# travisturner/pilosa

Hardware: AMD Instinct MI355X
Metric: PQL queries/sec (Count(Intersect(Row,Row))) on 1M-row x 1B-col set field (higher is better)
Workload: dtype bitmap(u64 words); 1 GPU; model=set field f, 1M-row x 1B-col (954 shards), global_batch=4096, seq_len=1000000000, parallelism=shard-range x1

## Files before the change

### pilosa_amd/kernels/binding.cpp

```cpp
#include <ATen/hip/HIPContext.h>
#include <torch/extension.h>

#include <pybind11/numpy.h>
#include <pybind11/stl.h>

#include <algorithm>
#include <cstring>
#include <mutex>
#include <vector>

#include "kernels.h"

namespace {

void check_dev(const torch::Tensor& t, const char* name) {
  TORCH_CHECK(t.is_cuda(), name, " must be a device tensor");
  TORCH_CHECK(t.is_contiguous(), name, " must be contiguous");
}

hipStream_t cur_stream(const torch::Tensor& t) {
  return at::hip::getCurrentHIPStream(t.device().index()).stream();
}

void check_launch(const char* what) {
// ... 340 lines not shown
  b.view = int32_t(a[0]);
  b.depth = int32_t(a[1]);
  TORCH_CHECK(b.depth >= 0 && b.depth <= 63, "bsi depth");
  TORCH_CHECK(a[0] >= 0 && a[0] < views.numel() / int64_t(sizeof(pk::ViewDev)), "bsi view slot");
  TORCH_CHECK(planes >= 1 && planes <= 64 && gchunk >= 1 && gchunk < (int64_t(1) << 31), "bsi_group_sum: slab / chunk");
  b.row_exists = a[2];
  b.row_sign = a[3];
  for (int i = 0; i < 64; i++) b.bit_row[i] = i < 63 ? a[4 + i] : -1;
  const int nslab = pk::launch_bsi_group_sum(
      reinterpret_cast<const pk::QueryProg*>(progs.data_ptr<uint8_t>()), int(G),
      reinterpret_cast<const pk::ViewDev*>(views.data_ptr<uint8_t>()), int(S), b, int(planes), int(gchunk),
      int(fmode), reinterpret_cast<unsigned long long*>(out_sum.data_ptr<int64_t>()),
      reinterpret_cast<unsigned long long*>(out_cnt.data_ptr<int64_t>()), cur_stream(progs));
  TORCH_CHECK(nslab >= 0, "bsi_group_sum: grid too large");
  check_launch("bsi_group_sum");
  return nslab;
}

void and2_count(torch::Tensor progs, torch::Tensor views, int64_t S, torch::Tensor pairs, torch::Tensor partial,
                int64_t cq, int64_t variant) {
  check_dev(progs, "progs");
  check_dev(views, "views");
  check_dev(pairs, "pairs");
  check_dev(partial, "partial");
  const int Q = int(progs.numel() / sizeof(pk::QueryProg));
  const int64_t n = int64_t(Q) * S * 16;
  TORCH_CHECK(pairs.numel() * pairs.element_size() >= n * 8, "pairs scratch must hold S*16*Q uint2");
  TORCH_CHECK(partial.scalar_type() == torch::kInt32 && partial.numel() >= n, "partial must be int32[S*16*Q]");
  pk::launch_and2_pairs(reinterpret_cast<const pk::QueryProg*>(progs.data_ptr<uint8_t>()), Q,
                        reinterpret_cast<const pk::ViewDev*>(views.data_ptr<uint8_t>()), int(S),
                        reinterpret_cast<uint2*>(pairs.data_ptr()), partial.data_ptr<int32_t>(), int(cq),
                        int(variant), cur_stream(progs));
  check_launch("and2_pairs");
}

pk::ViewDev viewdev_from(const torch::Tensor& vd);

void twin_build(torch::Tensor view, int64_t S, torch::Tensor rows, torch::Tensor twin) {
  check_dev(rows, "rows");
  check_dev(twin, "twin");
  TORCH_CHECK(rows.scalar_type() == torch::kInt32, "rows must be int32[R]");
  const int64_t R = rows.numel();
  TORCH_CHECK(R >= 0 && R < (int64_t(1) << 20) && S > 0, "twin_build sizes");
  TORCH_CHECK(twin.scalar_type() == torch::kInt64 && twin.numel() == R * S * 16 * 1024,
              "twin must be int64[R*S*16*1024]");
  pk::ViewDev v = viewdev_from(view);
  pk::launch_twin_build(v, int(S), rows.data_ptr<int32_t>(), int(R), reinterpret_cast<uint64_t*>(twin.data_ptr<int64_t>()),
                          cur_stream(twin));
  check_launch("twin_build");
}

void partial_sum_scatter(torch::Tensor partial, int64_t U, int64_t n, torch::Tensor ti, torch::Tensor out) {
  check_dev(partial, "partial");
  check_dev(ti, "ti");
  check_dev(out, "out");
  TORCH_CHECK(partial.scalar_type() == torch::kInt32 && partial.is_contiguous() && partial.numel() >= U * n,
              "partial must be int32[U*n]");
  TORCH_CHECK(ti.scalar_type() == torch::kInt64 && ti.numel() == n, "ti must be int64[n]");
  TORCH_CHECK(out.scalar_type() == torch::kInt64, "out must be int64");
  TORCH_CHECK(n < (int64_t(1) << 31) && U < (int64_t(1) << 40), "partial_sum_scatter sizes");
  pk::launch_partial_sum_scatter(partial.data_ptr<int32_t>(), U, int(n), ti.data_ptr<int64_t>(),
                                 out.data_ptr<int64_t>(), out.numel(), cur_stream(partial));
  check_launch("partial_sum_scatter");
}

pk::ViewDev viewdev_from(const torch::Tensor& vd) {
// ... 653 lines not shown
  const pk::ViewDev v = viewdev_from(view);
  check_dev(out, "out");
  TORCH_CHECK(out.scalar_type() == torch::kInt64, "out int64[n]");
  TORCH_CHECK(unit.dim() == 2 && unit.size(0) == 1, "block_dump takes one unit");
  if (out.numel() == 0) return;
  const torch::Tensor du = checked_units(unit, v, S, M, e, rows);
  pk::launch_block_dump(v, du.data_ptr<int32_t>(), int(M), int(e), rows.data_ptr<int64_t>(),
                        reinterpret_cast<uint64_t*>(out.data_ptr<int64_t>()), out.numel(), cur_stream(rows));
  check_launch("block_dump");
}

}

PYBIND11_MODULE(TORCH_EXTENSION_NAME, m) {
  m.doc() = "gfx950 HIP kernels for the bitmap index";
  m.attr("QUERYPROG_BYTES") = int(sizeof(pk::QueryProg));
  m.attr("VIEWDEV_BYTES") = int(sizeof(pk::ViewDev));
  m.attr("PAIR_VARIANTS") = std::vector<int>{63};
  m.attr("MAXLEAF") = pk::MAXLEAF;
  m.attr("MAXPROG") = pk::MAXPROG;
  m.def("expr_count", &expr_count, "batched boolean-expression count over all local shards",
        py::arg("progs"), py::arg("views"), py::arg("S"), py::arg("out"), py::arg("per_key"), py::arg("mode") = 0,
        py::arg("per_shard") = py::none());
  m.def("expr_materialize", &expr_materialize, "write result containers for a batch of expressions");
#ifdef PK_KBENCH
  m.attr("KBENCH") = true;
#else
  m.attr("KBENCH") = false;
#endif
  m.def("partial_sum_scatter", &partial_sum_scatter, "out[ti[q]] += column sums of int32[U][n] partials");
  m.def("and2_count", &and2_count, "Count(Intersect(a,b)) batch via key-major pair kernels", py::arg("progs"),
        py::arg("views"), py::arg("S"), py::arg("pairs"), py::arg("partial"), py::arg("cq") = 0,
        py::arg("variant") = 1);
  m.def("bsi_range", &bsi_range, "BSI predicate -> bitmap container per (shard, key)");
  m.def("bsi_range_count", &bsi_range_count, "Count(Row(v <op> x)): fused BSI predicate + count");
  m.def("bsi_minmax", &bsi_minmax, "BSI min/max descents per (shard, key); which: 0 both, 1 Min, 2 Max",
        py::arg("progs"), py::arg("views"), py::arg("S"), py::arg("bsi_args"), py::arg("out"), py::arg("which") = 0);
  m.def("bsi_kth_init", &bsi_kth_init, "Percentile: candidate tiles (exists & filter) and N, Nneg");
  m.def("bsi_kth_steps", &bsi_kth_steps, "Percentile: one descent launch per bit, MSB first");
  m.def("bsi_kth_replay", &bsi_kth_replay, "Percentile: host replay of the bit counts -> (magnitude, count)");
  m.def("bsi_distinct", &bsi_distinct, "Distinct: mark the magnitudes of exists & filter in the pos / neg bitmaps");
  m.def("distinct_slots", [](int64_t depth, int64_t want) { return int64_t(pk::distinct_slots(int(depth), int(want))); },
        "Distinct: tile slots per workgroup the launcher uses for this depth and request");
  m.def("leaf_src", &leaf_src, "src containers of plain rows straight from the arena (TopN srcs)");
  m.def("row_counts", &row_counts, "row counts of (shard, dense row) entries (device rank caches)");
  m.def("topn_cache_counts", &topn_cache_counts, "cache-only TopN: [candidate x shard] row counts");
  m.def("topn_cache_batch", &topn_cache_batch, "cache-only TopN batch: membership, totals, per-query top-n");
  m.def("mesh_cache_issue", &mesh_cache_issue, "mesh cache-only TopN share: params, partial buffer (pre all-reduce)");
  m.def("mesh_cache_finish", &mesh_cache_finish, "mesh cache-only TopN: select, D2H, decode (post all-reduce)");
  py::class_<CacheTopN>(m, "CacheTopN")
      .def(py::init<torch::Tensor, torch::Tensor, torch::Tensor, torch::Tensor, int64_t, torch::Tensor>())
      .def("run", &CacheTopN::run, "cache-only TopN batch end to end: (ids, counts, offsets) or None")
      .def_property_readonly("U", &CacheTopN::U)
      .def_property_readonly("stride", &CacheTopN::stride);
  m.def("upload_i32", &upload_i32, "small host int32 array -> device through a pinned ring (current stream)");
  m.def("topn_cache_partial", &topn_cache_partial, "mesh cache-only TopN: one rank's membership + partial totals");
  m.def("topn_cache_select32", &topn_cache_select32, "mesh cache-only TopN: per-query top-n of the reduced buffer");
  m.def("row_counts_sum", &row_counts_sum, "ids= re-count without src: per id the sum of shard row counts >= threshold");
  m.def("twin_build", &twin_build, "bitmap twins of dense array rows for the pair kernels");
  m.def("keymask_build", &keymask_build, "key-presence mask of every (shard, row) of a view");
  m.def("topn_hot_meta", &topn_hot_meta, "key-j container of every hot cache rank of the TopN index");
  m.def("topn_index", &topn_index, "build pass of the device TopN slot index (count or fill)");
  m.def("bsi_minmax_fold", &bsi_minmax_fold, "fold BSI min/max descents into one (value, count, found)");
  m.def("topn_src", &topn_src, "src-filtered TopN over the slot index: mode 1 heap walk, mode 2/3 ids= re-count (rebuilt / kept histograms)");
  m.def("bitgemm", &bitgemm, "row-pair intersection count matrix of dense bit rows (mode 1 MFMA i8, 0 VALU); "
        "c_split_stride > 0: one matrix per K-split; skip_lower: no tiles below the diagonal (A is B)",
        py::arg("A"), py::arg("B"), py::arg("M"), py::arg("N"), py::arg("KW"), py::arg("splits"), py::arg("mode"),
// ... 24 lines not shown
```

### pilosa_amd/kernels/kernels.h

```cpp
#pragma once
#include <hip/hip_runtime.h>
#include <stdint.h>

namespace pk {

constexpr int MAXLEAF = 16;
constexpr int MAXPROG = 32;
constexpr int ARRAY_MAX = 4096;
constexpr int RUN_MAX = 2048;
constexpr int CT_ARRAY = 1, CT_BITMAP = 2, CT_RUN = 3;
constexpr int OP_AND = 32, OP_OR = 33, OP_XOR = 34, OP_ANDNOT = 35;

__host__ __device__ __forceinline__ int meta_j(int64_t m) { return int(m & 15); }
__host__ __device__ __forceinline__ int meta_type(int64_t m) { return int((m >> 4) & 3); }
__host__ __device__ __forceinline__ int meta_n(int64_t m) { return int((m >> 6) & 0x1ffff); }
__host__ __device__ __forceinline__ int64_t meta_off16(int64_t m) { return int64_t(uint64_t(m) >> 23); }

struct QueryProg {
  int32_t nleaf;
  int32_t nprog;
  int32_t leaf_view[MAXLEAF];
  int64_t leaf_row[MAXLEAF];
  uint8_t prog[MAXPROG];
  int64_t pad[3];
// ... 5 lines not shown
  const int64_t* shard_base;
  const int64_t* meta;
  const uint16_t* payload;
  int64_t D;
  const uint16_t* keymask;
  uint64_t reserved0;
  uint64_t reserved1;
  const uint64_t* twin;
  const int32_t* twin_slot;
  int64_t twin_cutoff;
  const int32_t* hot_counts;
  const int32_t* hot_slot;
  const uint8_t* hot_valid;
  int64_t hot_h;
};
static_assert(sizeof(ViewDev) == 120, "ViewDev layout");

struct BsiArgs {
  int32_t view;
  int32_t depth;
  int64_t row_exists;
  int64_t row_sign;
  int64_t bit_row[64];
};

void launch_expr_count(const QueryProg* progs, int Q, const ViewDev* views, int S, unsigned long long* out,
                       int32_t* per_key, int64_t* per_shard, int mode, hipStream_t st);
void launch_expr_materialize(const QueryProg* progs, int Q, const ViewDev* views, int S, const int32_t* counts,
                             const int64_t* offs, uint16_t* outp, hipStream_t st);
void launch_partial_sum_scatter(const int32_t* partial, int64_t U, int n, const int64_t* ti, int64_t* out,
                                int64_t nout, hipStream_t st);
void launch_and2_pairs(const QueryProg* progs, int Q, const ViewDev* views, int S, uint2* pairs, int32_t* partial,
                       int cq, int variant, hipStream_t st);
void launch_bsi_range(const ViewDev* views, int S, BsiArgs bsi, int op, int64_t p1, int64_t p2, uint16_t* out_payload,
                      int64_t* out_meta, unsigned long long* out_count, hipStream_t st);
void launch_bsi_minmax_fold(const int64_t* o, int F, int G, int is_min, int64_t* out, int64_t* part,
                            hipStream_t st);
void launch_bsi_minmax(const QueryProg* progs, const ViewDev* views, int S, BsiArgs bsi, int64_t* out,
                       hipStream_t st, int which = 0);
__host__ __device__ inline int kth_chain(int largest_first, uint64_t c1, uint64_t& r, uint64_t& tot) {
  const uint64_t c0 = tot - c1;
  if (largest_first) {
    if (r < c1) { tot = c1; return 1; }
    r -= c1; tot = c0; return 0;
  }
  if (r < c0) { tot = c0; return 0; }
  r -= c0; tot = c1; return 1;
}
constexpr int KTH_CNT = 2 + 64;
void launch_bsi_kth_init(const QueryProg* progs, const ViewDev* views, int S, BsiArgs bsi, uint64_t* cand,
                         unsigned long long* cnt, hipStream_t st);
void launch_bsi_kth_step(const ViewDev* views, int S, BsiArgs bsi, uint64_t* cand, unsigned long long* cnt, int i,
                         uint64_t r, uint64_t tot, int largest_first, hipStream_t st);
void launch_bsi_sum(const QueryProg* progs, int Q, const ViewDev* views, int S, BsiArgs bsi,
                    unsigned long long* out_sum, unsigned long long* out_cnt, int fmode, hipStream_t st);
constexpr int GS_MAX_PLANES = 13;
int launch_bsi_group_sum(const QueryProg* progs, int G, const ViewDev* views, int S, BsiArgs bsi, int planes,
                         int gchunk, int fmode, unsigned long long* out_sum, unsigned long long* out_cnt,
                         hipStream_t st);

constexpr int DISTINCT_MAX_PLANES = 32;
int distinct_slots(int depth, int want);
int launch_bsi_distinct(const QueryProg* progs, const ViewDev* views, int S, BsiArgs bsi, int slots, int mark,
                        uint32_t* pos, uint32_t* neg, hipStream_t st);

int64_t launch_row_filter_counts(const ViewDev& fv, const ViewDev* xv, int64_t xd, int S, int64_t rows_per_block,
// ... 86 lines not shown
```

### pilosa_amd/kernels/pair_kernels.hip

```cpp
#include <hip/hip_runtime.h>
#include <stdint.h>

#include "kernels.h"
#include "device_util.h"

namespace pk {
namespace {

constexpr uint32_t NONE = 0xffffffffu;
constexpr uint32_t PRECOUNTED = 0xfffffffeu;

__global__ __launch_bounds__(256) void keymask_build_kernel(ViewDev v, int S, uint16_t* __restrict__ out) {
  const int64_t t = int64_t(blockIdx.x) * blockDim.x + threadIdx.x;
  if (t >= int64_t(S) * v.D) return;
  const int s = int(t / v.D);
  const int64_t d = t - int64_t(s) * v.D;
  v.keymask = nullptr;
  int64_t lo;
  out[t] = uint16_t(row_keys(v, s, d, lo));
}

__global__ __launch_bounds__(256) void pair_build_kernel(const QueryProg* __restrict__ progs, int Q,
                                                         const ViewDev* __restrict__ views, int S,
                                                         uint2* __restrict__ pairs, int hot) {
  const int64_t t = int64_t(blockIdx.x) * blockDim.x + threadIdx.x;
  if (t >= int64_t(Q) * S) return;
  const int s = int(t / Q), q = int(t % Q);
  const QueryProg& qp = progs[q];
  uint2* dst = pairs + int64_t(s) * 16 * Q + q;
  if (hot && qp.leaf_view[0] == qp.leaf_view[1] && qp.leaf_row[0] >= 0 && qp.leaf_row[1] >= 0) {
    const ViewDev& hv = views[qp.leaf_view[0]];
    if (hv.hot_counts != nullptr && gp(hv.hot_valid)[s]) {
      const int sa = gp(hv.hot_slot)[qp.leaf_row[0]], sb = gp(hv.hot_slot)[qp.leaf_row[1]];
      if (sa >= 0 && sb >= 0) {
        const int64_t h = hv.hot_h;
        const uint32_t c = uint32_t(gp(hv.hot_counts)[(int64_t(s) * h + min(sa, sb)) * h + max(sa, sb)]);
        dst[0] = make_uint2(PRECOUNTED, c);
#pragma unroll
        for (int j = 1; j < 16; j++) dst[int64_t(j) * Q] = make_uint2(NONE, NONE);
        return;
      }
    }
  }
  int64_t loa, lob;
  const uint32_t pa = row_keys(views[qp.leaf_view[0]], s, qp.leaf_row[0], loa);
  const uint32_t pb = row_keys(views[qp.leaf_view[1]], s, qp.leaf_row[1], lob);
  const uint32_t both = pa & pb;
#pragma unroll
  for (int j = 0; j < 16; j++) {
    uint2 e = make_uint2(NONE, NONE);
    if ((both >> j) & 1) {
      const uint32_t below = (1u << j) - 1;
      e.x = uint32_t(loa + __popc(pa & below));
      e.y = uint32_t(lob + __popc(pb & below));
    }
    dst[int64_t(j) * Q] = e;
  }
}


__device__ __forceinline__ void lds_clear(uint64_t* lb) {
  ulong2* l2 = reinterpret_cast<ulong2*>(lb);
  const int lane = wave_lane();
#pragma unroll
  for (int i = 0; i < 8; i++) l2[i * 64 + lane] = make_ulong2(0, 0);
}

template <bool BST = false>
__device__ __forceinline__ void stage(uint64_t* lb, const uint16_t* p, int64_t m) {
  const int lane = wave_lane();
  const int type = meta_type(m);
  ulong2* l2 = reinterpret_cast<ulong2*>(lb);
  if (type == CT_BITMAP) {
    const auto g = gp(reinterpret_cast<const ulong2*>(p));
    ulong2 t[8];
#pragma unroll
    for (int i = 0; i < 8; i++) t[i] = g[i * 64 + lane];
#pragma unroll
    for (int i = 0; i < 8; i++) l2[i * 64 + lane] = t[i];
    lds_fence();
    return;
  }
  uint32_t* l32 = reinterpret_cast<uint32_t*>(lb);
  if (BST && type == CT_ARRAY) {
    const int n = meta_n(m);
    const auto p4 = gp(reinterpret_cast<const uint4*>(p));
    const int n8 = (n + 7) >> 3;
    bool cleared = false;
    for (int b = 0; b < n8; b += 4 * 64) {
      uint4 v[4];
// ... 287 lines not shown
  const int lane = wave_lane();
  ulong2* dst = reinterpret_cast<ulong2*>(twin + w * 1024);
  const int64_t d = rows[r];
  int64_t c = -1;
  if (d >= 0) {
    int64_t lo;
    const uint32_t pres = row_keys(v, s, d, lo);
    if ((pres >> j) & 1) c = lo + __popc(pres & ((1u << j) - 1));
  }
  if (c < 0) {
#pragma unroll
    for (int i = 0; i < 8; i++) dst[i * 64 + lane] = make_ulong2(0, 0);
    return;
  }
  const int64_t m = gp(v.meta)[c];
  stage<true>(lb, payload_of(v, m), m);
  const ulong2* l2 = reinterpret_cast<const ulong2*>(lb);
#pragma unroll
  for (int i = 0; i < 8; i++) dst[i * 64 + lane] = l2[i * 64 + lane];
}

__device__ __forceinline__ int64_t meta_as_bitmap(int64_t m) {
  return (m & ~(int64_t(3) << 4)) | (int64_t(CT_BITMAP) << 4);
}

__device__ __forceinline__ void twin_swap(const ViewDev& v, int64_t d, int S, int64_t u, int64_t& m, uint64_t& pl) {
  if (v.twin_slot == nullptr || meta_type(m) != CT_ARRAY || meta_n(m) <= v.twin_cutoff) return;
  const int sl = gp(v.twin_slot)[d];
  if (sl < 0) return;
  pl = reinterpret_cast<uint64_t>(v.twin + ((int64_t(sl) * S + (u >> 4)) * 16 + (u & 15)) * 1024);
  m = meta_as_bitmap(m);
}

template <int CQ, bool BST = false, int TWN = 0>
__global__ __launch_bounds__(64, 5) void and2_pairs_v6_kernel(const QueryProg* __restrict__ progs, int Q,
                                                             const ViewDev* __restrict__ views, int S,
                                                             const uint2* __restrict__ pairs,
                                                             int32_t* __restrict__ partial) {
  __shared__ uint64_t lb[1024];
  const int lane = wave_lane();
  const int64_t gw = int64_t(xcd_remap(blockIdx.x, gridDim.x));
  const int nch = (Q + CQ - 1) / CQ;
  const int64_t u = gw / nch;
  if (u >= int64_t(S) * 16) return;
  const int q0 = int(gw % nch) * CQ;
  const int nq = min(CQ, Q - q0);

  uint32_t ea = NONE;
  int vai = -1;
  int64_t ma = 0, mb = 0;
  uint64_t pal = 0, pbl = 0;
  int mine = 0;
  if (lane < nq) {
    const uint2 e = pairs[u * Q + q0 + lane];
    if (e.x == PRECOUNTED) {
      mine = int(e.y);
    } else if (e.x != NONE) {
      ea = e.x;
      vai = progs[q0 + lane].leaf_view[0];
      const int vbi = progs[q0 + lane].leaf_view[1];
      ma = gp(views[vai].meta)[e.x];
      mb = gp(views[vbi].meta)[e.y];
      pal = reinterpret_cast<uint64_t>(payload_of(views[vai], ma));
      pbl = reinterpret_cast<uint64_t>(payload_of(views[vbi], mb));
      if (TWN & 1) twin_swap(views[vai], progs[q0 + lane].leaf_row[0], S, u, ma, pal);
      if (TWN & 2) twin_swap(views[vbi], progs[q0 + lane].leaf_row[1], S, u, mb, pbl);
    }
  }
  uint64_t todo = __ballot(ea != NONE);
  if (todo) {
    uint32_t cached = NONE;
    int cached_v = -1;
    int i = __builtin_ctzll(todo);
    todo &= todo - 1;
// ... 11 lines not shown
      int c = 0;
      if (a == cached && va == cached_v) {
        c = count_vs_head(lb, pB, mB, head);
      } else {
        const bool next_same = j >= 0 && __builtin_amdgcn_readlane(ea, j) == a &&
                               __builtin_amdgcn_readlane(vai, j) == va;
        if (!next_same && tA == CT_BITMAP && tB == CT_BITMAP) {
          c = and_global_bitmaps(reinterpret_cast<const uint64_t*>(pA), reinterpret_cast<const uint64_t*>(pB));
        } else if (!next_same && tA == CT_ARRAY && tB == CT_BITMAP && meta_n(mA) <= SMALL_ARRAY_N) {
          c = probe_small(gp(reinterpret_cast<const uint32_t*>(pB)), pA, meta_n(mA));
        } else if (!next_same && tA == CT_ARRAY && tB == CT_BITMAP) {
          lds_fence();
          stage<BST>(lb, pB, mB);
          cached = NONE;
          cached_v = -1;
          c = count_vs_lds(lb, pA, mA);
        } else {
          lds_fence();
          stage<BST>(lb, pA, mA);
          cached = a;
          cached_v = va;
          c = count_vs_head(lb, pB, mB, head);
        }
      }
      c = wave_sum(c);
      if (lane == i) mine = c;
      if (j < 0) break;
      i = j;
      todo &= todo - 1;
    }
  }
  if (lane < nq) partial[u * Q + q0 + lane] = mine;
}
}

void launch_twin_build(const ViewDev& v, int S, const int32_t* rows, int R, uint64_t* twin, hipStream_t st) {
  const int64_t w = int64_t(R) * S * 16;
  if (w <= 0) return;
  const dim3 grid(unsigned(w < 65535 ? w : 65535), unsigned((w + 65534) / 65535));
  hipLaunchKernelGGL(twin_build_kernel, grid, dim3(64), 0, st, v, S, rows, R, twin);
}

void launch_keymask_build(const ViewDev& v, int S, uint16_t* out, hipStream_t st) {
  const int64_t n = int64_t(S) * v.D;
  if (n == 0) return;
  hipLaunchKernelGGL(keymask_build_kernel, dim3(unsigned((n + 255) / 256)), dim3(256), 0, st, v, S, out);
}

template <int CQ, bool BST, int TWN>
void launch_v6(const QueryProg* progs, int Q, const ViewDev* views, int S, const uint2* pairs, int32_t* partial,
               hipStream_t st) {
  const int64_t wv = int64_t(S) * 16 * ((Q + CQ - 1) / CQ);
  hipLaunchKernelGGL((and2_pairs_v6_kernel<CQ, BST, TWN>), dim3(unsigned(wv)), dim3(64), 0, st, progs, Q, views, S,
                     pairs, partial);
}

void launch_and2_pairs(const QueryProg* progs, int Q, const ViewDev* views, int S, uint2* pairs, int32_t* partial,
                       int cq, int variant, hipStream_t st) {
  const int64_t items = int64_t(Q) * S;
  if (items == 0) return;
  const bool twin = variant == 63 && (cq > 0 ? cq == 64 : Q > 2048);
  if (variant == 63 && !twin) variant = 6;
  if (variant == 6 && cq <= 0 && Q <= 128) {
    variant = 39;
    cq = Q <= 32 ? 4 : (Q <= 64 ? 32 : 16);
  }
  if (cq <= 0) cq = Q <= 128 ? 8 : (Q <= 2048 ? 32 : 64);
  const int hot = variant == 6 || variant == 39 || variant == 63;
  hipLaunchKernelGGL(pair_build_kernel, dim3(unsigned((items + 255) / 256)), dim3(256), 0, st, progs, Q, views, S,
                     pairs, hot);
#define PK_LAUNCH(CQV)                                                         \
  if (variant == 39)                                                           \
    launch_v6<CQV, true, 0>(progs, Q, views, S, pairs, partial, st);           \
  else                                                                         \
    launch_v6<CQV, false, 0>(progs, Q, views, S, pairs, partial, st);          \
  break;
  switch (twin ? 0 : cq) {
    case 0: launch_v6<64, false, 3>(progs, Q, views, S, pairs, partial, st); break;
    case 4: PK_LAUNCH(4)
    case 8: PK_LAUNCH(8)
    case 16: PK_LAUNCH(16)
    case 32: PK_LAUNCH(32)
    default: PK_LAUNCH(64)
  }
#undef PK_LAUNCH
}

__global__ __launch_bounds__(256) void partial_sum_scatter_kernel(const int32_t* __restrict__ partial, int64_t U,
                                                                  int n, const int64_t* __restrict__ ti,
                                                                  unsigned long long* __restrict__ out,
                                                                  int64_t nout) {
  __shared__ long long acc[4][64];
  const int tx = threadIdx.x & 63, ty = threadIdx.x >> 6;
  const int q = int(blockIdx.x) * 64 + tx;
  const int64_t r0 = int64_t(blockIdx.y) * 128;
  const int64_t r1 = r0 + 128 < U ? r0 + 128 : U;
  long long a = 0;
  if (q < n) {
#pragma unroll 8
    for (int64_t r = r0 + ty; r < r1; r += 4) a += partial[r * n + q];
  }
  acc[ty][tx] = a;
  __syncthreads();
  if (ty == 0 && q < n) {
    const long long t = acc[0][tx] + acc[1][tx] + acc[2][tx] + acc[3][tx];
    const int64_t o = ti[q];
    if (t && o >= 0 && o < nout) atomicAdd(out + o, (unsigned long long)t);
  }
}

void launch_partial_sum_scatter(const int32_t* partial, int64_t U, int n, const int64_t* ti, int64_t* out,
                                int64_t nout, hipStream_t st) {
  if (U <= 0 || n <= 0) return;
  const dim3 grid(unsigned((n + 63) / 64), unsigned((U + 127) / 128));
  hipLaunchKernelGGL(partial_sum_scatter_kernel, grid, dim3(256), 0, st, partial, U, n, ti,
                     reinterpret_cast<unsigned long long*>(out), nout);
}

}
```

### pilosa_amd/ops/device.py

```python
from __future__ import annotations

import math
import os
import threading
import time
from dataclasses import dataclass, field
from typing import Dict, List, Optional, Sequence, Tuple

import numpy as np

from pilosa_amd.utils import tracing

MAXLEAF = 16
MAXPROG = 32
OP_AND, OP_OR, OP_XOR, OP_ANDNOT = 32, 33, 34, 35
KIND_AND2, KIND_ROW, KIND_GENERIC, KIND_FLAT, KIND_UNION = 0, 1, 2, 3, 4
KIND_ALIAS = 5
_KERNEL_MODE = {KIND_ROW: 1, KIND_GENERIC: 0, KIND_FLAT: 2, KIND_UNION: 3}


def flat_mask(progs: np.ndarray) -> np.ndarray:
    pg = progs["prog"].astype(np.int32)
    n = progs["nprog"].astype(np.int64)
    pos = np.arange(pg.shape[1])
# ... 1055 lines not shown

def hot_table_passable(table_rows_gen: int, table_gen: int, rows_gen: int, generation: int) -> bool:
    return table_rows_gen == rows_gen and table_gen == generation


def hot_stale_shards(snapshot: np.ndarray, shard_gen: np.ndarray) -> np.ndarray:
    return np.flatnonzero(np.asarray(snapshot) != np.asarray(shard_gen)).astype(np.int64)


def shard_runs(shards, block: int):
    out = []
    for s in np.asarray(shards, np.int64).tolist():
        if out and out[-1][1] == s and s - out[-1][0] < block:
            out[-1][1] = s + 1
        else:
            out.append([s, s + 1])
    return [(a, b) for a, b in out]



class DeviceRowBlock:

    __slots__ = ("shards", "counts", "offs", "payload", "spill")

    def __init__(self, shards, counts, offs, payload, spill=None):
        self.shards, self.counts, self.offs, self.payload, self.spill = list(shards), counts, offs, payload, spill

    def host(self):
        return (self.counts.cpu().numpy(), self.offs.cpu().numpy(), self.payload.cpu().numpy().view(np.uint16))


class GpuEngine:

    def __init__(self, device):
        import torch

        self.torch = torch
        self.device = torch.device(device)
        self.ext = kernels()
        self.copy_stream = torch.cuda.Stream(self.device) if self.device.type == "cuda" else None
        self.use_and2 = os.environ.get("PILOSA_AND2", "1") != "0"
        self.and2_cq = int(os.environ.get("PILOSA_AND2_CQ", "0"))
        self.and2_variant = int(os.environ.get("PILOSA_AND2_VARIANT", "6"))
        built = set(getattr(kernels(), "PAIR_VARIANTS", ()))
        self.use_twin = os.environ.get("PILOSA_TWIN", "1") != "0" and 63 in built
        self.use_hot = os.environ.get("PILOSA_HOTPAIR", "1") != "0"
        self.use_union = os.environ.get("PILOSA_UNION_KERNEL", "1") != "0"
        self.union_variant = int(os.environ.get("PILOSA_UNION_VARIANT", "2"))

    def _and2_aux(self, views: List["DeviceView"], n: int) -> int:
        if self.use_hot and self.and2_variant in (6, 39, 63):
            for v in views:
                v.ensure_hot()
        wave64 = self.and2_cq == 64 or (self.and2_cq <= 0 and n > 2048)
        if self.use_twin and wave64 and self.and2_variant in (6, 63) and \
                any([v.ensure_twin() for v in views]):
            return 2
        return 0

    def _views_tensor(self, views: List["DeviceView"]):
        arr = np.zeros(len(views), dtype=VIEWDEV_DTYPE)
        for i, v in enumerate(views):
            arr[i] = v.viewdev(hot=self.use_hot)
        key = arr.tobytes()
        memo = self.__dict__.setdefault("_vt_memo", {})
        hit = memo.get(key)
        torch = self.torch
        cuda = self.device.type == "cuda"
        if hit is not None:
            t, ev = hit
            if cuda:
                cur = torch.cuda.current_stream(self.device)
                cur.wait_event(ev)
                t.record_stream(cur)
            return t
        t = self._h2d(arr.view(np.uint8))
        ev = None
        if cuda:
            ev = torch.cuda.Event()
# ... 83 lines not shown
            is_row = is_row | is_and2
            is_and2 = np.zeros_like(is_and2)
        flat = flat_mask(progs)
        kind = np.where(is_and2, KIND_AND2, np.where(is_row, KIND_ROW,
                                                      np.where(flat, KIND_FLAT, KIND_GENERIC)))
        pos = np.arange(pg.shape[1])
        is_op = (pos[None, :] % 2 == 0) & (pos[None, :] > 0) & (pos[None, :] < np_[:, None])
        all_or = np.where(is_op, pg == OP_OR, True).all(axis=1)
        if self.use_union:
            kind = np.where((kind == KIND_FLAT) & all_or, KIND_UNION, kind)
        if is_and2.any():
            progs = self._hot_leaf_first(progs, is_and2)
            lr = progs["leaf_row"]
            for v in views:
                v.ensure_keymask()
        shd = self._and2_aux(views, int(is_and2.sum())) if is_and2.any() else 0
        varr = np.zeros(len(views), dtype=VIEWDEV_DTYPE)
        for i, v in enumerate(views):
            varr[i] = v.viewdev(hot=self.use_hot)
        host = [varr.view(np.uint8)]
        meta = []
        for k in (KIND_AND2, KIND_ROW, KIND_FLAT, KIND_UNION, KIND_GENERIC):
            sel = np.nonzero(kind == k)[0]
            if len(sel) == 0:
                continue
            if sort and len(sel) > 1:
                sel = sel[np.lexsort((lr[sel, 1], lr[sel, 0]))]
            host.append(np.ascontiguousarray(progs[sel]).view(np.uint8))
            host.append(sel.astype(np.int64))
            meta.append((k, len(sel)))
        dev = self._h2d_many(host)
        tv = dev[0]
        parts = [(dev[1 + 2 * i], dev[2 + 2 * i].view(torch.int64), k, n) for i, (k, n) in enumerate(meta)]
        return (Q, S, tv, parts, shd)

    def prepare_planned(self, Q: int, segs, buf: np.ndarray, views: List["DeviceView"], S: int):
        torch = self.torch
        if not S or not Q:
            return (Q, S, None, [])
        shd = 0
        n_and2 = sum(int(n) for kind, n, _, _ in segs if int(kind) == KIND_AND2)
        if n_and2:
            for v in views:
                v.ensure_keymask()
            shd = self._and2_aux(views, n_and2)
        varr = np.zeros(len(views), dtype=VIEWDEV_DTYPE)
        for i, v in enumerate(views):
            varr[i] = v.viewdev(hot=self.use_hot)
        tv, tb = self._h2d_many([varr.view(np.uint8), buf])
        parts = []
        for kind, n, po, oo in segs:
            if int(kind) == KIND_ALIAS:
                parts.append((tb[po:po + n * 8].view(torch.int64), tb[oo:oo + n * 8].view(torch.int64), KIND_ALIAS,
                              int(n)))
                continue
            parts.append((tb[po:po + n * QPROG_DTYPE.itemsize], tb[oo:oo + n * 8].view(torch.int64), int(kind), int(n)))
        return (Q, S, tv, parts, shd)

    @staticmethod
    def _hot_leaf_first(progs: np.ndarray, sel: np.ndarray) -> np.ndarray:
        lr = progs["leaf_row"]
        lv = progs["leaf_view"]
        idx = np.nonzero(sel)[0]
        keys = np.concatenate([lv[idx, 0].astype(np.int64) << 40 | lr[idx, 0], lv[idx, 1].astype(np.int64) << 40 | lr[idx, 1]])
        uniq, inv, cnt = np.unique(keys, return_inverse=True, return_counts=True)
        ca, cb = cnt[inv[:len(idx)]], cnt[inv[len(idx):]]
        swap = idx[(cb > ca) | ((cb == ca) & (keys[len(idx):] < keys[:len(idx)]))]
        if len(swap):
            progs = progs.copy()
            for f in ("leaf_row", "leaf_view"):
                col = progs[f]
                col[swap, 0], col[swap, 1] = col[swap, 1].copy(), col[swap, 0].copy()
        return progs

    def _and2_partial(self, tp, tv, S: int, n: int, shd: int = 0):
        torch = self.torch
        pairs = torch.empty(S * 16 * n * 2, dtype=torch.int32, device=self.device)
        partial = torch.empty(S * 16 * n, dtype=torch.int32, device=self.device)
        variant = self.and2_variant
        if variant == 6 and shd == 2 and self.use_twin:
            variant = 63
        self.ext.and2_count(tp, tv, S, pairs, partial, self.and2_cq, variant)
        return partial.view(S, 16, n)

    def to_host(self, t):
        with tracing.span("GpuEngine.d2h", gpu=True):
            return self._to_host(t)

    def _to_host(self, t):
        torch = self.torch
        if t.device.type != "cuda":
            return t
        h = torch.empty(t.shape, dtype=t.dtype, pin_memory=True)
        h.copy_(t, non_blocking=True)
        ev = torch.cuda.Event()
        ev.record()
        if _D2H_POLL:
            while not ev.query():
                time.sleep(_D2H_POLL)
        else:
            ev.synchronize()
        return h

    def launch_count(self, handle):
        with tracing.span("GpuEngine.launchCount", gpu=True, queries=handle[0], shards=handle[1]):
            return self._launch_count(handle)

    def _launch_count(self, handle):
        torch = self.torch
        Q, S, tv, parts = handle[:4]
        shd = len(handle) > 4 and handle[4]
        out = torch.zeros(Q, dtype=torch.int64, device=self.device)
        for tp, ti, kind, n in parts:
            if kind == KIND_ALIAS:
                out.index_copy_(0, ti, out.index_select(0, tp))
                continue
            if kind == KIND_AND2:
                self.ext.partial_sum_scatter(self._and2_partial(tp, tv, S, n, shd).view(-1), S * 16, n, ti, out)
                continue
            else:
                o = torch.zeros(n, dtype=torch.int64, device=self.device)
                mode = _KERNEL_MODE[kind]
                if kind == KIND_UNION and self.union_variant == 2:
                    mode = 4
                self.ext.expr_count(tp, tv, S, o, None, mode)
            out.index_copy_(0, ti, o)
        return out

    def count_per_shard(self, exprs: Sequence[object]) -> np.ndarray:
        progs, views, S = self.compile_batch(exprs)
        return self.count_per_shard_progs(progs, views, S)

    @staticmethod
    def pair_programs(slot_a: int, dense_a: np.ndarray, slot_b: int, dense_b: np.ndarray) -> np.ndarray:
        dense_a = np.broadcast_to(np.asarray(dense_a, np.int64), np.shape(dense_b)) if np.ndim(dense_a) == 0 \
            else np.asarray(dense_a, np.int64)
        dense_b = np.asarray(dense_b, np.int64)
        Q = len(dense_b)
        p = np.zeros(Q, dtype=QPROG_DTYPE)
        p["nleaf"] = 2
        p["nprog"] = 3
        p["leaf_view"][:, 0] = slot_a
        p["leaf_view"][:, 1] = slot_b
        p["leaf_row"][:, 0] = dense_a
        p["leaf_row"][:, 1] = dense_b
        p["prog"][:, 0] = 0
        p["prog"][:, 1] = 1
        p["prog"][:, 2] = OP_AND
# ... 469 lines not shown
```

Measured before the change: 648,700 queries/s.

## Answer hot-table AND2 queries from count table and compact remainder on device

Adds a device-side split kernel that sorts each Count(Intersect) query by whether both rows have slots in the view's precomputed hot pair-count table. Hot queries are summed straight from that table across shards. The other queries are compacted, and the pair-build, v6 pair and scatter kernels read the live query count from device memory and exit early for the unused grid. This avoids running the full pair grid for queries the table already answers, at the cost of a single-workgroup serial split kernel and extra launches. Any block of this kind should be ordered before dependent launches, and the path is on by default for batches of at least 512 queries when hot tables exist.

```diff
diff --git a/pilosa_amd/kernels/binding.cpp b/pilosa_amd/kernels/binding.cpp
--- a/pilosa_amd/kernels/binding.cpp
+++ b/pilosa_amd/kernels/binding.cpp
@@ -396,6 +396,41 @@
                         reinterpret_cast<uint2*>(pairs.data_ptr()), partial.data_ptr<int32_t>(), int(cq),
                         int(variant), cur_stream(progs));
   check_launch("and2_pairs");
+}
+
+void and2_count_total(torch::Tensor progs, torch::Tensor views, int64_t S, torch::Tensor ti, torch::Tensor out,
+                      torch::Tensor pairs, torch::Tensor partial, torch::Tensor work, int64_t cq, int64_t variant) {
+  check_dev(progs, "progs");
+  check_dev(views, "views");
+  check_dev(ti, "ti");
+  check_dev(out, "out");
+  check_dev(pairs, "pairs");
+  check_dev(partial, "partial");
+  check_dev(work, "work");
+  TORCH_CHECK(progs.numel() % int64_t(sizeof(pk::QueryProg)) == 0 &&
+                  reinterpret_cast<uintptr_t>(progs.data_ptr()) % 16 == 0,
+              "progs must hold whole programs, 16-byte aligned");
+  TORCH_CHECK(views.numel() % int64_t(sizeof(pk::ViewDev)) == 0, "views must hold whole ViewDev records");
+  const int64_t Q = progs.numel() / int64_t(sizeof(pk::QueryProg));
+  const int64_t V =views.numel() / int64_t(sizeof(pk::ViewDev));
+  TORCH_CHECK(Q < (int64_t(1) << 31) && S > 0 && S < (int64_t(1) << 27) && V > 0 && V < (int64_t(1) << 31),
+              "and2_count_total: batch size");
+  const int64_t n = Q * S * 16;
+  TORCH_CHECK(ti.scalar_type() == torch::kInt64 && ti.numel() == Q, "ti must be int64[Q]");
+  TORCH_CHECK(out.scalar_type() == torch::kInt64 && out.is_contiguous(), "out must be int64");
+  TORCH_CHECK(pairs.numel() * pairs.element_size() >= n * 8, "pairs scratch must hold S*16*Q uint2");
+  TORCH_CHECK(partial.scalar_type() == torch::kInt32 && partial.numel() >= n, "partial must be int32[S*16*Q]");
+  TORCH_CHECK(work.scalar_type() == torch::kUInt8 && work.is_contiguous() &&
+                  work.numel() >= pk::and2_work_bytes(Q) && reinterpret_cast<uintptr_t>(work.data_ptr()) % 256 == 0,
+              "work must be 256-byte aligned uint8[and2_work_bytes(Q)]");
+  const bool ok = pk::launch_and2_total(
+      reinterpret_cast<const pk::QueryProg*>(progs.data_ptr<uint8_t>()), int(Q),
+      reinterpret_cast<const pk::ViewDev*>(views.data_ptr<uint8_t>()), int(V), int(S), ti.data_ptr<int64_t>(),
+      out.data_ptr<int64_t>(), out.numel(), reinterpret_cast<uint2*>(pairs.data_ptr()), partial.data_ptr<int32_t>(),
+      work.data_ptr<uint8_t>(), int(cq), int(variant), cur_stream(progs));
+  TORCH_CHECK(ok, "and2_count_total: no device-count pair kernel for ", Q, " queries, cq ", cq, ", variant ",
+              variant);
+  check_launch("and2_count_total");
 }
 
 pk::ViewDev viewdev_from(const torch::Tensor& vd);
@@ -1115,7 +1150,11 @@
   m.def("and2_count", &and2_count, "Count(Intersect(a,b)) batch via key-major pair kernels", py::arg("progs"),
         py::arg("views"), py::arg("S"), py::arg("pairs"), py::arg("partial"), py::arg("cq") = 0,
         py::arg("variant") = 1);
-  m.def("bsi_range", &bsi_range, "BSI predicate -> bitmap container per (shard, key)");
+  m.def("and2_count_total", &and2_count_total,
+        "Count(Intersect(a,b)) totals into out[ti]: table-answered queries compacted out of the pair grid");
+  m.def("and2_work_bytes", [](int64_t Q) { return pk::and2_work_bytes(Q); },
+        "bytes of and2_count_total's work scratch for Q queries");
+  m.def("bsi_range",&bsi_range, "BSI predicate -> bitmap container per (shard, key)");
   m.def("bsi_range_count", &bsi_range_count, "Count(Row(v <op> x)): fused BSI predicate + count");
   m.def("bsi_minmax", &bsi_minmax, "BSI min/max descents per (shard, key); which: 0 both, 1 Min, 2 Max",
         py::arg("progs"), py::arg("views"), py::arg("S"), py::arg("bsi_args"), py::arg("out"), py::arg("which") = 0);
diff --git a/pilosa_amd/kernels/kernels.h b/pilosa_amd/kernels/kernels.h
--- a/pilosa_amd/kernels/kernels.h
+++ b/pilosa_amd/kernels/kernels.h
@@ -61,6 +61,11 @@
                                 int64_t nout, hipStream_t st);
 void launch_and2_pairs(const QueryProg* progs, int Q, const ViewDev* views, int S, uint2* pairs, int32_t* partial,
                        int cq, int variant, hipStream_t st);
+constexpr int64_t AND2_WORK_HEAD = 256;
+inline int64_t and2_work_bytes(int64_t Q) { return AND2_WORK_HEAD + Q * int64_t(sizeof(QueryProg) + 16 + 8); }
+bool launch_and2_total(const QueryProg* progs, int Q, const ViewDev* views, int V, int S, const int64_t* ti,
+                       int64_t* out, int64_t nout, uint2* pairs, int32_t* partial, uint8_t* work, int cq,
+                       int variant, hipStream_t st);
 void launch_bsi_range(const ViewDev* views, int S, BsiArgs bsi, int op, int64_t p1, int64_t p2, uint16_t* out_payload,
                       int64_t* out_meta, unsigned long long* out_count, hipStream_t st);
 void launch_bsi_minmax_fold(const int64_t* o, int F, int G, int is_min, int64_t* out, int64_t* part,
diff --git a/pilosa_amd/kernels/pair_kernels.hip b/pilosa_amd/kernels/pair_kernels.hip
--- a/pilosa_amd/kernels/pair_kernels.hip
+++ b/pilosa_amd/kernels/pair_kernels.hip
@@ -20,9 +20,9 @@
   out[t] = uint16_t(row_keys(v, s, d, lo));
 }
 
-__global__ __launch_bounds__(256) void pair_build_kernel(const QueryProg* __restrict__ progs, int Q,
-                                                         const ViewDev* __restrict__ views, int S,
-                                                         uint2* __restrict__ pairs, int hot) {
+__device__ __forceinline__ void pair_build_body(const QueryProg* __restrict__ progs, int Q,
+                                                const ViewDev* __restrict__ views, int S,
+                                                uint2* __restrict__ pairs, int hot) {
   const int64_t t = int64_t(blockIdx.x) * blockDim.x + threadIdx.x;
   if (t >= int64_t(Q) * S) return;
   const int s = int(t / Q), q = int(t % Q);
@@ -56,6 +56,19 @@
     }
     dst[int64_t(j) * Q] = e;
   }
+}
+
+__global__ __launch_bounds__(256) void pair_build_kernel(const QueryProg* __restrict__ progs, int Q,
+                                                         const ViewDev* __restrict__ views, int S,
+                                                         uint2* __restrict__ pairs, int hot) {
+  pair_build_body(progs, Q, views, S, pairs, hot);
+}
+
+__global__ __launch_bounds__(256) void pair_build_dq_kernel(const QueryProg* __restrict__ progs,
+                                                            const int32_t* __restrict__ nq,
+                                                            const ViewDev* __restrict__ views, int S,
+                                                            uint2* __restrict__ pairs, int hot) {
+  pair_build_body(progs, *nq, views, S, pairs, hot);
 }
 
 
@@ -409,14 +422,32 @@
   m = meta_as_bitmap(m);
 }
 
-template <int CQ, bool BST = false, int TWN = 0>
-__global__ __launch_bounds__(64, 5) void and2_pairs_v6_kernel(const QueryProg* __restrict__ progs, int Q,
+template <bool DQ>
+struct QCount {
+  int q;
+  __device__ __forceinline__ int get() const { return q; }
+};
+template <>
+struct QCount<true> {
+  const int32_t* q;
+  __device__ __forceinline__ int get() const { return *q; }
+};
+
+template <int CQ, bool BST = false, int TWN = 0, bool DQ = false>
+__global__ __launch_bounds__(64, 5) void and2_pairs_v6_kernel(const QueryProg* __restrict__ progs, QCount<DQ> qc,
                                                              const ViewDev* __restrict__ views, int S,
                                                              const uint2* __restrict__ pairs,
                                                              int32_t* __restrict__ partial) {
   __shared__ uint64_t lb[1024];
   const int lane = wave_lane();
-  const int64_t gw = int64_t(xcd_remap(blockIdx.x, gridDim.x));
+  const int Q = qc.get();
+  uint32_t nblk = gridDim.x;
+  if (DQ) {
+    const int64_t live = int64_t(S) * 16 * ((Q + CQ - 1) / CQ);
+    if (int64_t(blockIdx.x) >= live) return;
+    nblk = uint32_t(live);
+  }
+  const int64_t gw = int64_t(xcd_remap(blockIdx.x, nblk));
   const int nch = (Q + CQ - 1) / CQ;
   const int64_t u = gw / nch;
   if (u >= int64_t(S) * 16) return;
@@ -494,6 +525,109 @@
   }
   if (lane < nq) partial[u * Q + q0 + lane] = mine;
 }
+
+constexpr int SPLIT_T = 1024, SPLIT_W = SPLIT_T / 64, SPLIT_MAXV = 64;
+
+__global__ __launch_bounds__(SPLIT_T) void pair_split_kernel(const QueryProg* __restrict__ progs, int Q,
+                                                             const ViewDev* __restrict__ views, int V, int S,
+                                                             const int64_t* __restrict__ ti,
+                                                             QueryProg* __restrict__ lprogs,
+                                                             int64_t* __restrict__ lti, int4* __restrict__ hotl,
+                                                             int32_t* __restrict__ cnt) {
+  __shared__ int vok[SPLIT_MAXV];
+  __shared__ int wl[SPLIT_W], wh[SPLIT_W];
+  __shared__ int dst[SPLIT_T];
+  const int tid = threadIdx.x, lane = tid & 63, wv = tid >> 6;
+  const int nv = min(V, SPLIT_MAXV);
+  if (tid < nv)
+    vok[tid] = views[tid].hot_counts != nullptr && views[tid].hot_slot != nullptr && views[tid].hot_valid != nullptr;
+  __syncthreads();
+  for (int v = 0; v < nv; v++) {
+    if (!vok[v]) continue;
+    const auto hv = gp(views[v].hot_valid);
+    for (int s = tid; s < S; s += SPLIT_T)
+      if (!hv[s]) vok[v] = 0;
+  }
+  __syncthreads();
+  int lbase = 0, hbase = 0;
+  for (int q0 = 0; q0 < Q; q0 += SPLIT_T) {
+    const int q = q0 + tid;
+    bool hot = false;
+    int4 he = make_int4(0, 0, 0, 0);
+    if (q < Q) {
+      const QueryProg& qp = progs[q];
+      const int va = qp.leaf_view[0];
+      const int64_t ra = qp.leaf_row[0], rb = qp.leaf_row[1];
+      if (va == qp.leaf_view[1] && va >= 0 && va < nv && vok[va] && ra >= 0 && rb >= 0) {
+        const auto hs = gp(views[va].hot_slot);
+        const int sa = hs[ra], sb = hs[rb];
+        if (sa >= 0 && sb >= 0) {
+          hot = true;
+          he = make_int4(va, min(sa, sb), max(sa, sb), q);
+        }
+      }
+    }
+    const bool live = q < Q && !hot;
+    const uint64_t bl = __ballot(live), bh = __ballot(hot);
+    if (lane == 0) {
+      wl[wv] = __popcll(bl);
+      wh[wv] = __popcll(bh);
+    }
+    __syncthreads();
+    int pl = 0, ph = 0, tl = 0, th = 0;
+#pragma unroll
+    for (int w = 0; w < SPLIT_W; w++) {
+      pl += w < wv ? wl[w] : 0;
+      ph += w < wv ? wh[w] : 0;
+      tl += wl[w];
+      th += wh[w];
+    }
+    const uint64_t below = (1ull << lane) - 1;
+    int d = -1;
+    if (live) {
+      d = lbase + pl + __popcll(bl & below);
+      lti[d] = ti[q];
+    }
+    if (hot) hotl[hbase + ph + __popcll(bh & below)] = he;
+    dst[tid] = d;
+    __syncthreads();
+    const uint4* src = reinterpret_cast<const uint4*>(progs + q0);
+    uint4* out = reinterpret_cast<uint4*>(lprogs);
+    const int n16 = min(SPLIT_T, Q - q0) * int(sizeof(QueryProg) / 16);
+    for (int i = tid; i < n16; i += SPLIT_T) {
+      const int dq = dst[i >> 4];
+      if (dq >= 0) out[int64_t(dq) * 16 + (i & 15)] = src[i];
+    }
+    __syncthreads();
+    lbase += tl;
+    hbase += th;
+  }
+  if (tid == 0) {
+    cnt[0] = lbase;
+    cnt[1] = hbase;
+  }
+}
+static_assert(sizeof(QueryProg) == 16 * 16, "pair_split_kernel copies a program as 16 uint4");
+
+__global__ __launch_bounds__(256) void hot_pair_sum_kernel(const ViewDev* __restrict__ views, int S,
+                                                           const int4* __restrict__ hotl,
+                                                           const int32_t* __restrict__ cnt,
+                                                           const int64_t* __restrict__ ti,
+                                                           unsigned long long* __restrict__ out, int64_t nout) {
+  const int w = int(blockIdx.x) * 4 + int(threadIdx.x >> 6);
+  if (w >= cnt[1]) return;
+  const int lane = wave_lane();
+  const int4 e = hotl[w];
+  const ViewDev& hv = views[e.x];
+  const int64_t h = hv.hot_h;
+  const auto hc = gp(hv.hot_counts) + int64_t(e.y) * h + e.z;
+  int64_t a = 0;
+#pragma unroll 4
+  for (int s = lane; s < S; s += 64) a += uint32_t(hc[int64_t(s) * h * h]);
+  a = wave_sum_i64(a);
+  const int64_t o = ti[e.w];
+  if (lane == 0 && a && o >= 0 && o < nout) atomicAdd(out + o, (unsigned long long)a);
+}
 }
 
 void launch_twin_build(const ViewDev& v, int S, const int32_t* rows, int R, uint64_t* twin, hipStream_t st) {
@@ -513,8 +647,16 @@
 void launch_v6(const QueryProg* progs, int Q, const ViewDev* views, int S, const uint2* pairs, int32_t* partial,
                hipStream_t st) {
   const int64_t wv = int64_t(S) * 16 * ((Q + CQ - 1) / CQ);
-  hipLaunchKernelGGL((and2_pairs_v6_kernel<CQ, BST, TWN>), dim3(unsigned(wv)), dim3(64), 0, st, progs, Q, views, S,
-                     pairs, partial);
+  hipLaunchKernelGGL((and2_pairs_v6_kernel<CQ, BST, TWN>), dim3(unsigned(wv)), dim3(64), 0, st, progs, QCount<false>{Q},
+                     views, S, pairs, partial);
+}
+
+template <int CQ, int TWN>
+void launch_v6_dq(const QueryProg* progs, int Q, const int32_t* nq, const ViewDev* views, int S, const uint2* pairs,
+                  int32_t* partial, hipStream_t st) {
+  const int64_t wv = int64_t(S) * 16 * ((Q + CQ - 1) / CQ);
+  hipLaunchKernelGGL((and2_pairs_v6_kernel<CQ, false, TWN, true>), dim3(unsigned(wv)), dim3(64), 0, st, progs,
+                     QCount<true>{nq}, views, S, pairs, partial);
 }
 
 void launch_and2_pairs(const QueryProg* progs, int Q, const ViewDev* views, int S, uint2* pairs, int32_t* partial,
@@ -548,10 +690,9 @@
 #undef PK_LAUNCH
 }
 
-__global__ __launch_bounds__(256) void partial_sum_scatter_kernel(const int32_t* __restrict__ partial, int64_t U,
-                                                                  int n, const int64_t* __restrict__ ti,
-                                                                  unsigned long long* __restrict__ out,
-                                                                  int64_t nout) {
+__device__ __forceinline__ void partial_sum_scatter_body(const int32_t* __restrict__ partial, int64_t U, int n,
+                                                         const int64_t* __restrict__ ti,
+                                                         unsigned long long* __restrict__ out, int64_t nout) {
   __shared__ long long acc[4][64];
   const int tx = threadIdx.x & 63, ty = threadIdx.x >> 6;
   const int q = int(blockIdx.x) * 64 + tx;
@@ -571,6 +712,23 @@
   }
 }
 
+__global__ __launch_bounds__(256) void partial_sum_scatter_kernel(const int32_t* __restrict__ partial, int64_t U,
+                                                                  int n, const int64_t* __restrict__ ti,
+                                                                  unsigned long long* __restrict__ out,
+                                                                  int64_t nout) {
+  partial_sum_scatter_body(partial, U, n, ti, out, nout);
+}
+
+__global__ __launch_bounds__(256) void partial_sum_scatter_dq_kernel(const int32_t* __restrict__ partial, int64_t U,
+                                                                     const int32_t* __restrict__ nq,
+                                                                     const int64_t* __restrict__ ti,
+                                                                     unsigned long long* __restrict__ out,
+                                                                     int64_t nout) {
+  const int n = *nq;
+  if (int(blockIdx.x) * 64 >= n) return;
+  partial_sum_scatter_body(partial, U, n, ti, out, nout);
+}
+
 void launch_partial_sum_scatter(const int32_t* partial, int64_t U, int n, const int64_t* ti, int64_t* out,
                                 int64_t nout, hipStream_t st) {
   if (U <= 0 || n <= 0) return;
@@ -579,4 +737,37 @@
                      reinterpret_cast<unsigned long long*>(out), nout);
 }
 
-}
+bool launch_and2_total(const QueryProg* progs, int Q, const ViewDev* views, int V, int S, const int64_t* ti,
+                       int64_t* out, int64_t nout, uint2* pairs, int32_t* partial, uint8_t* work, int cq,
+                       int variant, hipStream_t st) {
+  if (Q <= 128 || S <= 0 || V <= 0) return false;
+  const bool twin = variant == 63 && (cq > 0 ? cq == 64 : Q > 2048);
+  if (variant == 63 && !twin) variant = 6;
+  if (variant != 6 && !twin) return false;
+  if (cq <= 0) cq = Q <= 2048 ? 32 : 64;
+  if (cq != 32 && cq != 64) return false;
+  int32_t* cnt = reinterpret_cast<int32_t*>(work);
+  QueryProg* lprogs = reinterpret_cast<QueryProg*>(work + AND2_WORK_HEAD);
+  int4* hotl = reinterpret_cast<int4*>(work + AND2_WORK_HEAD + int64_t(Q) * sizeof(QueryProg));
+  int64_t* lti = reinterpret_cast<int64_t*>(work + AND2_WORK_HEAD + int64_t(Q) * (sizeof(QueryProg) + 16));
+  unsigned long long* o64 = reinterpret_cast<unsigned long long*>(out);
+  hipLaunchKernelGGL(pair_split_kernel, dim3(1), dim3(SPLIT_T), 0, st, progs, Q, views, V, S, ti, lprogs, lti, hotl,
+                     cnt);
+  hipLaunchKernelGGL(hot_pair_sum_kernel, dim3(unsigned((Q + 3) / 4)), dim3(256), 0, st, views, S, hotl, cnt, ti,
+                     o64, nout);
+  const int64_t items = int64_t(Q) * S;
+  hipLaunchKernelGGL(pair_build_dq_kernel, dim3(unsigned((items + 255) / 256)), dim3(256), 0, st, lprogs, cnt, views,
+                     S, pairs, 1);
+  if (twin)
+    launch_v6_dq<64, 3>(lprogs, Q, cnt, views, S, pairs, partial, st);
+  else if (cq == 64)
+    launch_v6_dq<64, 0>(lprogs, Q, cnt, views, S, pairs, partial, st);
+  else
+    launch_v6_dq<32, 0>(lprogs, Q, cnt, views, S, pairs, partial, st);
+  const int64_t U = int64_t(S) * 16;
+  const dim3 grid(unsigned((Q + 63) / 64), unsigned((U + 127) / 128));
+  hipLaunchKernelGGL(partial_sum_scatter_dq_kernel, grid, dim3(256), 0, st, partial, U, cnt, lti, o64, nout);
+  return true;
+}
+
+}
diff --git a/pilosa_amd/ops/device.py b/pilosa_amd/ops/device.py
--- a/pilosa_amd/ops/device.py
+++ b/pilosa_amd/ops/device.py
@@ -1111,6 +1111,8 @@
 
 class GpuEngine:
 
+    PAIR_COMPACT_MIN = 512
+
     def __init__(self, device):
         import torch
 
@@ -1124,6 +1126,8 @@
         built = set(getattr(kernels(), "PAIR_VARIANTS", ()))
         self.use_twin = os.environ.get("PILOSA_TWIN", "1") != "0" and 63 in built
         self.use_hot = os.environ.get("PILOSA_HOTPAIR", "1") != "0"
+        self.use_compact = os.environ.get("PILOSA_PAIR_COMPACT", "1") != "0"
+        self.PAIR_COMPACT_MIN = int(os.environ.get("PILOSA_PAIR_COMPACT_MIN", str(self.PAIR_COMPACT_MIN)))
         self.use_union = os.environ.get("PILOSA_UNION_KERNEL", "1") != "0"
         self.union_variant = int(os.environ.get("PILOSA_UNION_VARIANT", "2"))
 
@@ -1273,7 +1277,7 @@
         dev = self._h2d_many(host)
         tv = dev[0]
         parts = [(dev[1 + 2 * i], dev[2 + 2 * i].view(torch.int64), k, n) for i, (k, n) in enumerate(meta)]
-        return (Q, S, tv, parts, shd)
+        return (Q, S, tv, parts, shd, bool(varr["hot_counts"].any()))
 
     def prepare_planned(self, Q: int, segs, buf: np.ndarray, views: List["DeviceView"], S: int):
         torch = self.torch
@@ -1296,7 +1300,7 @@
                               int(n)))
                 continue
             parts.append((tb[po:po + n * QPROG_DTYPE.itemsize], tb[oo:oo + n * 8].view(torch.int64), int(kind), int(n)))
-        return (Q, S, tv, parts, shd)
+        return (Q, S, tv, parts, shd, bool(varr["hot_counts"].any()))
 
     @staticmethod
     def _hot_leaf_first(progs: np.ndarray, sel: np.ndarray) -> np.ndarray:
@@ -1324,6 +1328,20 @@
         self.ext.and2_count(tp, tv, S, pairs, partial, self.and2_cq, variant)
         return partial.view(S, 16, n)
 
+    def _compact_route(self, n: int) -> bool:
+        return self.use_compact and self.use_hot and self.and2_variant in (6, 63) and \
+            n > 128 and n >= self.PAIR_COMPACT_MIN and (self.and2_cq <= 0 or self.and2_cq in (32, 64))
+
+    def _and2_total(self, tp, tv, S: int, n: int, ti, out, shd: int = 0):
+        torch = self.torch
+        pairs = torch.empty(S * 16 * n * 2, dtype=torch.int32, device=self.device)
+        partial = torch.empty(S * 16 * n, dtype=torch.int32, device=self.device)
+        work = torch.empty(self.ext.and2_work_bytes(n), dtype=torch.uint8, device=self.device)
+        variant = self.and2_variant
+        if variant == 6 and shd == 2 and self.use_twin:
+            variant = 63
+        self.ext.and2_count_total(tp, tv, S, ti, out, pairs, partial, work, self.and2_cq, variant)
+
     def to_host(self, t):
         with tracing.span("GpuEngine.d2h", gpu=True):
             return self._to_host(t)
@@ -1351,10 +1369,14 @@
         torch = self.torch
         Q, S, tv, parts = handle[:4]
         shd = len(handle) > 4 and handle[4]
+        tabled = len(handle) > 5 and handle[5]
         out = torch.zeros(Q, dtype=torch.int64, device=self.device)
         for tp, ti, kind, n in parts:
             if kind == KIND_ALIAS:
                 out.index_copy_(0, ti, out.index_select(0, tp))
+                continue
+            if kind == KIND_AND2 and tabled and self._compact_route(n):
+                self._and2_total(tp, tv, S, n, ti, out, shd)
                 continue
             if kind == KIND_AND2:
                 self.ext.partial_sum_scatter(self._and2_partial(tp, tv, S, n, shd).view(-1), S * 16, n, ti, out)
```

Measured after the change: 710,600 queries/s (median of 6 runs). +9.5%, better.
